# sangyun884/HR-VITON

Hardware: AMD Instinct MI355X
Metric: 1024x768 try-on images/sec (train_generator.py step: tocg+glue, G fwd/bwd, D fwd/bwd x2, VGG, Adam) (higher is better)
Workload: dtype bf16; 1 GPU; BASELINE configs[3] (SURVEY 8d config #4, headline): train_generator.py 1024x768, 4 img/GPU, --fp16 (bf16 MFMA operands, fp32 accumulate), SPADE ng...; global_batch=4, height=1024, width=768, parallelism=dp1-allreduce, persistent_grid_cus=256, dist_backend=none (single process), world_size=1, rccl_ranks=0

## Files before the change

hr-viton_amd/_lib.py:

```python
from __future__ import annotations

import ctypes as C
import os

HERE = os.path.dirname(os.path.abspath(__file__))
LIB_PATH = os.path.join(HERE, "libhrviton_hip.so")

HRV_MAX_SRC = 4
ACT_NONE, ACT_RELU, ACT_LRELU, ACT_TANH = 0, 1, 2, 3


class hrv_src_t(C.Structure):
    _fields_ = [("ptr", C.c_void_p), ("C", C.c_int32), ("cstride", C.c_int32), ("coff", C.c_int32),
                ("up_shift", C.c_int32), ("pre_act", C.c_int32), ("C_real", C.c_int32)]


class hrv_spade_epi_t(C.Structure):
    _fields_ = [("x", C.c_void_p), ("x_cstride", C.c_int32), ("x_coff", C.c_int32), ("C", C.c_int32),
                ("_pad", C.c_int32), ("mean", C.c_void_p), ("rstd", C.c_void_p), ("noise_z", C.c_void_p),
                ("noise_scale", C.c_void_p), ("g1p_out", C.c_void_p)]


class hrv_norm_bwd_t(C.Structure):
    _fields_ = [("N", C.c_int32), ("H", C.c_int32), ("W", C.c_int32), ("C", C.c_int32),
# ... 60 lines not shown
                ("act", C.c_int32), ("act_slope", C.c_float),
                ("out", C.c_void_p), ("out_cstride", C.c_int32), ("out_coff", C.c_int32),
                ("actv", C.c_void_p), ("actv_cstride", C.c_int32), ("actv_coff", C.c_int32),
                ("x_up_channels", C.c_int32), ("x2", C.c_void_p), ("x2_cstride", C.c_int32), ("x2_coff", C.c_int32),
                ("tiles", C.c_void_p), ("gb_table", C.c_void_p), ("tiles_phase", C.c_int32)]


class hrv_conv_p2_t(C.Structure):
    _fields_ = [("N", C.c_int32), ("H", C.c_int32), ("W", C.c_int32), ("Cin", C.c_int32),
                ("src", C.c_void_p), ("src_cstride", C.c_int32), ("src_coff", C.c_int32), ("Cout", C.c_int32),
                ("w_packed", C.c_void_p), ("bias", C.c_void_p),
                ("act", C.c_int32), ("act_slope", C.c_float),
                ("mask", C.c_void_p), ("mask_cstride", C.c_int32), ("mask_coff", C.c_int32), ("mask_slope", C.c_float), ("out_f32", C.c_int32),
                ("out", C.c_void_p), ("out_cstride", C.c_int32), ("out_coff", C.c_int32),
                ("res_f32", C.c_int32), ("residual", C.c_void_p), ("res_cstride", C.c_int32), ("res_coff", C.c_int32),
                ("res_after_mask", C.c_int32)]


class hrv_conv_s2_t(C.Structure):
    _fields_ = [("mode", C.c_int32),
                ("N", C.c_int32), ("Hs", C.c_int32), ("Ws", C.c_int32), ("K", C.c_int32),
                ("src", C.c_void_p), ("src_cstride", C.c_int32), ("src_coff", C.c_int32),
                ("Ho", C.c_int32), ("Wo", C.c_int32), ("cols", C.c_int32), ("Cph", C.c_int32),
                ("w_packed", C.c_void_p), ("bias", C.c_void_p),
                ("act", C.c_int32), ("act_slope", C.c_float),
                ("out", C.c_void_p), ("out_cstride", C.c_int32), ("out_coff", C.c_int32), ("out_f32", C.c_int32),
                ("residual", C.c_void_p), ("res_cstride", C.c_int32), ("res_coff", C.c_int32), ("res_f32", C.c_int32),
                ("mask", C.c_void_p), ("mask_cstride", C.c_int32), ("mask_coff", C.c_int32), ("mask_slope", C.c_float)]


class hrv_s2_pack_job_t(C.Structure):
# ... 217 lines not shown
    "hrv_grid_sample_nchw_bwd_f32": (C.c_int, [_vp, _i32, _i32, _i32, _i32, _vp, _i32, _i32, _vp, _vp, _vp, _vp]),
    "hrv_softmax_nchw_f32": (C.c_int, [_vp, _i32, _i32, _i64, _vp, _vp]),
    "hrv_softmax_nchw_bwd_f32": (C.c_int, [_vp, _vp, _i32, _i32, _i64, _vp, _vp]),
    "hrv_cross_entropy_nchw_f32": (C.c_int, [_vp, _vp, _i32, _i32, _i64, _f, _vp, _vp, _vp, _vp]),
    "hrv_tapsum_bwd_nhwc_f32": (C.c_int, [_vp, _i32, _i32, _i32, _i32, _i32, _i32, _i32, _i32, _vp, _i32, _vp]),
    "hrv_tap_expand_nhwc": (C.c_int, [_vp, _i32, _i32, _i32, _i32, _i32, _i32, _i32, _i32, _i32, _i32, _vp, _vp]),
    "hrv_mul_f32": (C.c_int, [_vp, _vp, _i64, _vp, _vp]),
    "hrv_spade_gb_packed_bytes": (_i64, [_i32, _i32, _i32, _i32]),
    "hrv_spade_gb_supported": (C.c_int, [_i32, _i32, _i32, _i32, _i32, _i32, _i32]),
    "hrv_spade_gb_pack_dev": (C.c_int, [_i32, _vp, _vp, _i32, _i32, _i32, _vp, _vp]),
    "hrv_spade_gb_bf16": (C.c_int, [C.POINTER(hrv_spade_gb_t), _vp]),
    "hrv_conv_p2_packed_bytes": (C.c_int64, [_i32, _i32]),
    "hrv_conv_p2_supported": (C.c_int, [_i32, _i32, _i32, _i32, _i32]),
    "hrv_conv_p2_pack_dev": (C.c_int, [_i32, _vp, _vp, _i32, _i32, _vp, _f, _vp, _vp]),
    "hrv_conv_p2_bf16": (C.c_int, [C.POINTER(hrv_conv_p2_t), _vp]),
    "hrv_conv_s2_packed_bytes": (C.c_int64, [_i32, _i32, _i32]),
    "hrv_conv_s2_supported": (C.c_int, [_i32, _i32, _i32, _i32, _i32, _i32, _i32]),
    "hrv_conv_s2_pack_dev": (C.c_int, [_i32, _vp, _i32, _i32, _i32, _vp, _f, _vp, _vp]),
    "hrv_conv_s2_pack_multi_dev": (C.c_int, [_i32, C.POINTER(hrv_s2_pack_job_t), _vp]),
    "hrv_conv_s2_bf16": (C.c_int, [C.POINTER(hrv_conv_s2_t), _vp]),
    "hrv_space_to_depth2_cells_bf16": (C.c_int, [_vp, _i32, _i32, _i32, _i32, _i32, _i32, _i32, _i32, _i32, _vp, _vp]),
    "hrv_instnorm_apply_nhwc_bf16out": (C.c_int, [_vp, _i32, _i32, _i32, _i32, _i32, _i32, _vp, _vp, _i32, _f, _vp, _i32, _i32, _vp]),
    "hrv_scale_bf16": (C.c_int, [_vp, _i64, _f, _vp, _vp]),
    "hrv_split3_nhwc_bf16": (C.c_int, [_vp, _i64, _i32, _i32, _i32, _vp, _vp]),
    "hrv_pad_width_nhwc_bf16": (C.c_int, [_vp, _i64, _i32, _i32, _i32, _vp, _vp]),
    "hrv_spade_fused_packed_bytes": (C.c_int64, [_i32]),
    "hrv_spade_fused_supported": (C.c_int, [_i32, _i32, _i32, _i32, _i32, _i32]),
    "hrv_spade_fused_pack_dev": (C.c_int, [_vp, _vp, _i32, _vp, _vp, _i32, _vp, _vp]),
    "hrv_spade_fused_bf16": (C.c_int, [C.POINTER(hrv_spade_fused_t), _vp]),
    "hrv_spade_tiles_plan_bytes": (C.c_int64, [_i32, _i32, _i32]),
# ... 62 lines not shown
```

hr-viton_amd/csrc/conv_p2.hip:

```cpp
#include <string.h>

#include <type_traits>
#include <utility>

#include "patch_pass.h"

namespace hrv {

constexpr int P2_PW = 20;
constexpr int P2_PBUF = 23 * 1024;
constexpr int p2_sb(int ntp) { return ntp * 2048; }
constexpr int p2_patch_off(int ntp) { return 3 * p2_sb(ntp); }
constexpr int p2_cb_off(int ntp) { return p2_patch_off(ntp) + 2 * P2_PBUF; }
constexpr int p2_lds(int ntp) { return p2_cb_off(ntp) + 512; }
constexpr int p2_blocks_per_cu(int ntp) { return ntp == 1 ? 3 : 2; }
static_assert(2 * ((p2_lds(4) + 1279) / 1280) * 1280 <= 160 * 1024, "two blocks per CU");
static_assert(3 * ((p2_lds(1) + 1279) / 1280) * 1280 <= 160 * 1024, "three blocks per CU for single-tile passes");

struct P2Params {
  const void* src; int src_cs, src_co, Cin; unsigned src_bytes;
  int N, H, W;
  const void* wp; unsigned w_bytes;
  int npass;
  int ntp[PATCH_MAXP];
// ... 99 lines not shown
  const rsrc_t a_rsrc = make_rsrc(reinterpret_cast<const char*>(p.src) + (size_t)T.n * p.src_bytes, p.src_bytes);
  const rsrc_t w_rsrc = make_rsrc(p.wp, p.w_bytes);
#pragma unroll
  for (int k = 0; k < 6; ++k) p2_patch_piece<NTP>(p, smem, a_rsrc, T, 0, 0, k * 4 + wave, lane);
#pragma unroll
  for (int q = 0; q < 2; ++q)
#pragma unroll
    for (int k = 0; k < NBW; ++k) {
      int idx = wave + 4 * k;
      idx = idx < NPW ? idx : (NPW >= 4 ? idx - 4 : idx % NPW);
      dma16(w_rsrc, reinterpret_cast<float*>(smem + q * p2_sb(NTP) + idx * 1024), (unsigned)lane * 16u,
            p.woff[pass] + (unsigned)q * (unsigned)(NPW * 1024) + (unsigned)idx * 1024u);
    }
}

template <int NTP, int EPI>
__device__ __forceinline__ void p2_pass(const P2Params& p, unsigned char* const smem, const int pass, const PatchTile T, const int bid,
                                        const bool load_consts, const bool wait_all, const bool first, const bool last, const int nxt_pass,
                                        const PatchTile NT_) {
  const int tid = threadIdx.x, lane = tid & 63;
  const int wave = __builtin_amdgcn_readfirstlane(tid >> 6);
  const int l31 = lane & 31, lh = lane >> 5;
  constexpr int NPW = NTP * 2;
  constexpr int NBW = (NPW + 3) / 4;
  constexpr int NST = 4 * NTP;
  unsigned char* const ring = smem;
  float* const cbuf = reinterpret_cast<float*>(smem + p2_cb_off(NTP));
  const rsrc_t w_rsrc = make_rsrc(p.wp, p.w_bytes);
  const rsrc_t a_rsrc = make_rsrc(reinterpret_cast<const char*>(p.src) + (size_t)T.n * p.src_bytes, p.src_bytes);
  const unsigned wbase = p.woff[pass];
  const int tile0 = p.tile0[pass];
// ... 269 lines not shown
  }
  if (p.tlog && tid == 0 && last) {
    p.tlog[(size_t)bid * 8 + 7] = tl_pack;
    p.tlog[(size_t)bid * 8 + 6] = wall_clock64();
  }
}

template <int NTP, int EPI>
__global__ __launch_bounds__(256, p2_blocks_per_cu(NTP)) void conv_p2_kernel(const P2Params p, const int pass0, const int pass1) {
  __shared__ __attribute__((aligned(1024))) unsigned char smem[p2_lds(NTP)];
  const int lane = threadIdx.x & 63, wave = __builtin_amdgcn_readfirstlane((int)threadIdx.x >> 6);
#define P2_TILE(BID) patch_tile(BID, p.W, p.H, p.m_tiles)
#define P2_HEAD(PASS, T) p2_head<NTP>(p, PASS, smem, T, wave, lane)
#define P2_PASS(...) p2_pass<NTP, EPI>(p, smem, __VA_ARGS__)
  PATCH_PASS_UNITS(p, pass0, pass1, P2_TILE, P2_HEAD, P2_PASS, p.tlog)
#undef P2_TILE
#undef P2_HEAD
#undef P2_PASS
}

}

using namespace hrv;

extern "C" int64_t hrv_conv_p2_packed_bytes(int32_t Cin, int32_t Cout) {
  PatchPlan pl;
  if (!p2_plan(Cin, Cout, pl)) return -1;
  return pl.bytes;
}

// ... 42 lines not shown
  memset(&p, 0, sizeof(p));
  p.src = d->src; p.src_cs = d->src_cstride; p.src_co = d->src_coff; p.Cin = d->Cin; p.src_bytes = (unsigned)sbytes;
  p.N = d->N; p.H = d->H; p.W = d->W;
  p.wp = d->w_packed; p.w_bytes = (unsigned)pl.bytes;
  patch_plan_copy(p, pl);
  p.nchunk = (d->Cin + 31) / 32;
  p.m_tiles = (int)patch_tiles(d->N, d->H, d->W);
  p.Cout = d->Cout;
  p.bias = d->bias; p.act = d->act; p.slope = d->act_slope;
  p.res = d->residual; p.res_cs = d->res_cstride; p.res_co = d->res_coff; p.res_f32 = d->res_f32; p.res_after = d->res_after_mask;
  p.mask = d->mask; p.mask_cs = d->mask_cstride; p.mask_co = d->mask_coff; p.mask_slope = d->mask_slope;
  p.out = d->out; p.out_cs = d->out_cstride; p.out_co = d->out_coff; p.out_f32 = d->out_f32;
  p.tlog = diag_tlog(p.m_tiles);
  p.pp = patch_pp(p.m_tiles) ? 1 : 0;
  if (p.pp) p.tlog = nullptr;
  patch_pass_groups(pl, p.m_tiles, p.pp != 0, p2_blocks_per_cu, [&](const int a, const int b, const int grid) {
    const dim3 g3(grid), b3(256);
    const hipStream_t st = (hipStream_t)stream;
    const int epi = p.res ? 2 : (p.mask ? 1 : 0);
#define P2_LAUNCH(NTP_)                                                                                                 \
  {                                                                                                                     \
    if (epi == 0) hipLaunchKernelGGL((conv_p2_kernel<NTP_, 0>), g3, b3, 0, st, p, a, b);                                \
    else if (epi == 1) hipLaunchKernelGGL((conv_p2_kernel<NTP_, 1>), g3, b3, 0, st, p, a, b);                           \
    else hipLaunchKernelGGL((conv_p2_kernel<NTP_, 2>), g3, b3, 0, st, p, a, b);                                         \
  }
    if (pl.ntp[a] == 4) P2_LAUNCH(4)
    else if (pl.ntp[a] == 3) P2_LAUNCH(3)
    else if (pl.ntp[a] == 2) P2_LAUNCH(2)
    else P2_LAUNCH(1)
#undef P2_LAUNCH
// ... 4 lines not shown
```

hr-viton_amd/gen_train.py:

```python
from __future__ import annotations

import os
from typing import Dict, List, Optional, Sequence, Tuple

import torch
import torch.nn as nn

from . import _lib, ops
from . import train_ops as T
from .ops import ACT_LRELU, ACT_NONE, ACT_RELU, ACT_TANH, Act, _ceil4

Grads = Dict[nn.Parameter, torch.Tensor]


def attach_grad_sync(sync):
    for p in sync.params:
        p._hrv_grad_sync = sync


def detach_grad_sync(params):
    for p in params:
        if hasattr(p, "_hrv_grad_sync"):
            del p._hrv_grad_sync

# ... 200 lines not shown

    def forward(self, x: Act, actv: Optional[Act], z: Optional[torch.Tensor], save: bool = True, fused=None, stats=None):
        n = self.norm
        dev = x.t.device
        if fused is not None:
            sg, shift = fused
            zz = z
            if stats is not None:
                ns, (mean, rstd) = stats
            else:
                ns = self.vecs()[1] if zz is not None else None
                mean, rstd = ops.instnorm_stats(x, zz, ns if zz is not None else None)
            out = ops.alloc(x.N, x.H, x.W, self.C, dev, bf16=True)
            g1p = torch.empty((x.N, x.H, x.W, self.Cp), dtype=torch.bfloat16, device=dev) if save else None
            pk = T.spade_fused_pack(self.shared.wparam.data, self.shared.bparam.data, n.conv_gamma.weight.data, n.conv_beta.weight.data)
            T.spade_fused_forward(sg, shift, x, mean, rstd, zz, n.noise_scale.data, pk, n.conv_gamma.bias.data, n.conv_beta.bias.data,
                                  self.act, 0.2, out, g1p, actv if save else None, self.name + ".conv_shared+gamma|beta",
                                  tiles=T.spade_tile_plan_for(sg, shift, x.N, x.H, x.W))
            ctx = dict(x=x, z=zz, ns=ns, mean=mean, rstd=rstd, actv=actv, g1p=Act(g1p, self.C) if save else None, out=out)
            return out, ctx
        bc, ns = self.vecs()
        zz = z
        if stats is not None:
            mean, rstd = stats[1]
        else:
            mean, rstd = ops.instnorm_stats(x, zz, ns if zz is not None else None)
        mb = T.MMA_BF16[0]
        cfg = ops.engine_tile("mb", 0, self.G * 64, mb and actv.bf16, 3, 3, 1, 1, 1, 0, self.hid, x.N, x.H, x.W, wide=True,
                              base=None if mb else self.cfg)
        out_bf16 = mb and actv.bf16 and self.C % 8 == 0
        if (mb and actv.bf16 and out_bf16 and x.cstride % 4 == 0 and
                T.spade_gb_ok(0, self.C, self.Cp, self.hid, x.N, x.H, x.W)):
            out = ops.alloc(x.N, x.H, x.W, self.C, dev, bf16=True)
            g1p = torch.empty((x.N, x.H, x.W, self.Cp), dtype=torch.bfloat16, device=dev) if save else None
# ... 85 lines not shown
        with T.wgrad_side(dgb.N * dgb.H * dgb.W, dgb, actv):
            dwcat, db = _pair_slot(n.conv_gamma.weight, n.conv_beta.weight), _pair_slot(n.conv_gamma.bias, n.conv_beta.bias)
            if Cp != C_ or dwcat is None or db is None:
                dwcat = torch.empty((2 * Cp, self.hid, 3, 3), device=dev)
                db = torch.empty(2 * Cp, device=dev)
            T.conv_wgrad(dgb, actv, 0, 0, self.hid, 3, 3, 1, 1, dwcat, name=self.name + ".gb.wgrad", dbias=db)
            direct = flat_grad_slot(n.conv_gamma.weight) is not None
            keep = (lambda t: t) if direct else (lambda t: t.clone())
            _acc(grads, n.conv_gamma.weight, keep(dwcat[:C_]))
            _acc(grads, n.conv_beta.weight, keep(dwcat[Cp:Cp + C_]))
            _acc(grads, n.conv_gamma.bias, keep(db[:C_]))
            _acc(grads, n.conv_beta.bias, keep(db[Cp:Cp + C_]))
        if (Cp == C_ and T.MMA_BF16[0] and dgb.bf16 and actv.bf16 and dact.cstride % 8 == 0 and (2 * C_) % 32 == 0 and
                T.conv_p2_ok(2 * C_, self.hid, actv.N, actv.H, actv.W)):
            pk = T.conv_p2_pack(2, n.conv_gamma.weight.data, n.conv_beta.weight.data, 2 * C_, self.hid)
            T.conv_p2(dgb, pk, self.hid, dact, mask=actv, mask_slope=0.0, name=self.name + ".gb.dgrad",
                      flops=2.0 * actv.N * actv.H * actv.W * 2 * C_ * self.hid * 9, tag=" [spade_gb]")
        elif (Cp == C_ and T.MMA_BF16[0] and dgb.bf16 and actv.bf16 and
                T.spade_gb_ok(1, C_, Cp, self.hid, actv.N, actv.H, actv.W)):
            T.spade_gb_dgrad(dgb, T.spade_gb_pack(1, n.conv_gamma.weight.data, n.conv_beta.weight.data), C_, actv, 0.0, dact,
                             self.name + ".gb.dgrad")
        else:
            T.conv_dgrad(dgb, wcat, actv.H, actv.W, 1, 1, act_mask=actv, slope=0.0, out=dact, name=self.name + ".gb.dgrad",
                         batch=getattr(self.shared, "pack_batch", None) if Cp == C_ else None)


class BlockT:
    def __init__(self, blk: nn.Module, name: str):
        self.blk, self.name = blk, name
        self.learned = blk.learned_shortcut
        self.n0 = SpadeT(blk.norm_0, ACT_LRELU, name + ".norm_0")
        self.n1 = SpadeT(blk.norm_1, ACT_LRELU, name + ".norm_1")
# ... 38 lines not shown
        mb = T.MMA_BF16[0] and (seg.W >> seg_shift) % 4 == 0
        sg = seg
        if mb and seg.coff == 0 and seg.cstride == 8:
            sg = getattr(seg, "_as_bf16", None)
            if sg is None:
                sg = seg._as_bf16 = Act(seg.t.to(torch.bfloat16), seg.C)
        mb = mb and sg.bf16
        segx = ops.tap_expand(sg, seg_shift, 3)
        cp = sg.Cp
        wt_all, b_all = T.shared_taps_prep([n_.shared.wparam.data for n_ in norms], [n_.shared.bparam.data for n_ in norms], cp)
        hid = norms[0].hid
        actv_all = T.conv_forward_dev(wt_all, [(segx, 0)], 1, 0, shift=b_all, act=ACT_RELU,
                                      out_bf16=mb, name=self.name + ".conv_shared[x%d as 1x1 over taps]" % len(norms))
        return segx, [actv_all.slice(hid * i, hid) for i in range(len(norms))]

    def shared_backward(self, segx: Act, dact_all: Act, grads: Grads):
        norms = self.norms()
        hid, cp = norms[0].hid, segx.C // 9
        with T.wgrad_side(dact_all.N * dact_all.H * dact_all.W, dact_all, segx):
            dw = torch.empty((hid * len(norms), segx.C, 1, 1), device=dact_all.t.device)
            db = torch.empty(hid * len(norms), device=dact_all.t.device)
            T.conv_wgrad(dact_all, segx, 0, 0, segx.C, 1, 1, 1, 0, dw, name=self.name + ".conv_shared.wgrad", dbias=db)
            gws = [grad_buffer(n_.shared.wparam) for n_ in norms]
            gbs = [grad_buffer(n_.shared.bparam) for n_ in norms]
            T.shared_taps_grad(dw, db, gws, gbs, cp)
            for n_, gw, gb in zip(norms, gws, gbs):
                _acc(grads, n_.shared.wparam, gw)
                _acc(grads, n_.shared.bparam, gb)

    def forward(self, x: Act, seg: Act, seg_shift: int, zs, out: Optional[Act], out_up: int, out_act: int,
                save: bool = True):
        zi = iter(zs)
        ctx = {"x": x}
        sgf = self.fused_label_map(x, seg, seg_shift)
        fused = None
        if sgf is not None:
            fused = (sgf, seg_shift)
            norms = self.norms()
            hid = norms[0].hid
# ... 23 lines not shown
        h0, ctx["n0"] = self.n0.forward(x, next(ai), z_0, save, fused, st_0)
        dx = self.c0.forward([(h0, 0)])
        h1, ctx["n1"] = self.n1.forward(dx, next(ai), next(zi), save, fused)
        o = self.c1.forward([(h1, 0)], residual=x_s, act=out_act, out=out, out_up=out_up,
                            out_bf16=out is None and h1.bf16 and self.c1.conv.out_channels % 8 == 0)
        ctx.update(h0=h0, h1=h1)
        return o, ctx

    def backward(self, ctx, d_out: Act, grads: Grads) -> Act:
        x = ctx["x"]
        norms = self.norms()
        hid = norms[0].hid
        dact_all = ops.alloc(x.N, x.H, x.W, hid * len(norms), x.t.device,
                             bf16=bool(T.MMA_BF16[0] and ctx["segx"].bf16 and x.W % 4 == 0))
        k0 = 1 if self.learned else 0
        dh16 = bool(T.MMA_BF16[0] and os.environ.get("HRV_DH_BF16", "1") != "0")
        def down(conv, d_y, h, norm, nctx):
            slot = norm.dout_slot(nctx, dh16 and h.bf16)
            if slot is None:
                return conv.backward(d_y, [(h, 0)], grads, dx_bf16=dh16 and h.bf16), None
            dgb, dbeta, mask = slot
            conv.backward(d_y, [(h, 0)], grads, act_mask=mask, slope=0.2, dx_out=dbeta)
            return dbeta, dgb
        d_h1, dgb1 = down(self.c1, d_out, ctx["h1"], self.n1, ctx["n1"])
        d_dx = self.n1.backward(ctx["n1"], d_h1, grads, None, False, dact_all.slice(hid * (k0 + 1), hid), dx_bf16=True, dgb=dgb1)
        d_h0, dgb0 = down(self.c0, d_dx, ctx["h0"], self.n0, ctx["n0"])
        mode = os.environ.get("HRV_NORM_BWD2", "")
        d_hs = None
        if self.learned and mode != "0" and ctx["n0"]["z"] is not None and ctx["ns"]["z"] is not None and not x.bf16:
            d_hs, dgbs = down(self.cs, d_out, ctx["hs"], self.ns_, ctx["ns"])
            a0, as_ = self.n0.norm_args(ctx["n0"], d_h0), self.ns_.norm_args(ctx["ns"], d_hs)
            for a, dgb in ((a0, dgb0), (as_, dgbs)):
                if dgb is not None:
                    a.update(act=ACT_NONE, out=None, dgb=dgb)
            pair = T.norm_bwd2(x, a0, as_, only_where_faster=mode != "1")
            if pair is not None:
                d_x, dgb0, dgbs = pair
                self.n0.after_norm(ctx["n0"], dgb0, a0["dnoise_scale"], grads, dact_all.slice(hid * k0, hid))
                self.ns_.after_norm(ctx["ns"], dgbs, as_["dnoise_scale"], grads, dact_all.slice(0, hid))
                self.shared_backward(ctx["segx"], dact_all, grads)
                return d_x
        d_x = self.n0.backward(ctx["n0"], d_h0, grads, None, False, dact_all.slice(hid * k0, hid), dgb=dgb0)
        if self.learned:
            if d_hs is None:
                d_hs, dgbs = down(self.cs, d_out, ctx["hs"], self.ns_, ctx["ns"])
            self.ns_.backward(ctx["ns"], d_hs, grads, d_x, True, dact_all.slice(0, hid), dgb=dgbs)
        else:
            T.add_slice(d_out, d_x, True)
        self.shared_backward(ctx["segx"], dact_all, grads)
        return d_x


def noise_elems(gen: nn.Module, N: int) -> int:
    return sum((3 if getattr(gen, name).learned_shortcut else 2) * ((N * (gen.sw << j) * (gen.sh << j) + 3) // 4 * 4)
               for j, name in enumerate(gen._blocks()))


def noise_planes(gen: nn.Module, N: int, zall: torch.Tensor):
    out, off = {}, 0
    for j, name in enumerate(gen._blocks()):
        h, w = gen.sh << j, gen.sw << j
        zn = N * w * h
        planes = []
        for _ in range(3 if getattr(gen, name).learned_shortcut else 2):
# ... 723 lines not shown
```

hr-viton_amd/train_ops.py:

```python
from __future__ import annotations

import ctypes as C
import itertools
import os
from typing import Optional, Sequence, Tuple

import torch

from . import _lib, ops
from .conv_dispatch import (COUT1, MMA_BF16, P2, THIN, conv_p2_ok, plan_dgrad, plan_forward,
                            plan_wgrad, wgrad_desc)
from .ops import ACT_LRELU, ACT_NONE, ACT_RELU, Act, _ceil4, _stream, _Timed, _workspace


_FROZEN_PACKS: dict = {}


def evict_serving_packs(tokens):
    toks = set(tokens)
    dead = [k for k in _FROZEN_PACKS
            if any(isinstance(e, tuple) and len(e) == 3 and e[0] == "serve" and e[1] in toks for e in k)]
    for k in dead:
        del _FROZEN_PACKS[k]
    return len(dead)
# ... 1591 lines not shown
    nbytes = lib.hrv_conv_p2_packed_bytes(K, cols)
    assert nbytes > 0, (K, cols)
    buf = torch.empty(nbytes // 2, dtype=torch.bfloat16, device=w.device)
    _lib.check(lib.hrv_conv_p2_pack_dev(mode, w.data_ptr(), None if w2 is None else w2.data_ptr(), K, cols,
                                        None if sigma is None else sigma.data_ptr(), wscale, buf.data_ptr(), _stream()),
               "hrv_conv_p2_pack_dev")
    if key is not None:
        if len(_FROZEN_PACKS) > 256:
            _FROZEN_PACKS.clear()
        _FROZEN_PACKS[key] = (buf, ())
    return buf


def conv_p2(src: Act, packed: torch.Tensor, cols: int, out: Act, bias: Optional[torch.Tensor] = None, act: int = ACT_NONE, slope: float = 0.2,
            mask: Optional[Act] = None, mask_slope: float = 0.0, name: str = "conv", flops: float = 0.0, tag: str = "",
            residual: Optional[Act] = None, res_after_mask: bool = False, variant: str = ""):
    lib = _lib.load()
    assert src.bf16 and out.C == cols
    d = _lib.hrv_conv_p2_t()
    d.N, d.H, d.W, d.Cin = src.N, src.H, src.W, src.C
    d.src, d.src_cstride, d.src_coff, d.Cout = src.t.data_ptr(), src.cstride, src.coff, cols
    d.w_packed = packed.data_ptr()
    if bias is not None:
        d.bias = bias.data_ptr()
    d.act, d.act_slope = act, slope
    if mask is not None:
        assert mask.bf16 and mask.C == cols
        d.mask, d.mask_cstride, d.mask_coff, d.mask_slope = mask.t.data_ptr(), mask.cstride, mask.coff, mask_slope
    d.out, d.out_cstride, d.out_coff, d.out_f32 = out.t.data_ptr(), out.cstride, out.coff, 0 if out.bf16 else 1
    if residual is not None:
        assert residual.C == cols
        d.residual, d.res_cstride, d.res_coff, d.res_f32 = residual.t.data_ptr(), residual.cstride, residual.coff, 0 if residual.bf16 else 1
        d.res_after_mask = 1 if res_after_mask else 0
    nb = (ops.act_bytes(src) + ops.act_bytes(out) + (ops.act_bytes(mask) if mask is not None else 0.0) +
          (ops.act_bytes(residual) if residual is not None else 0.0) + 2.0 * src.C * cols * 9)
    with ops._Timed("conv", name + tag, flops, nb, "conv_p2_kernel", variant):
        _lib.check(lib.hrv_conv_p2_bf16(C.byref(d), _stream()), f"hrv_conv_p2_bf16[{name}]")
    return out


S2_FWD, S2_DGRAD, S2_CELLS = 0, 1, 2


def conv_s2_ok(mode: int, K: int, cols: int, Cph: int, N: int, Ho: int, Wo: int) -> bool:
    if os.environ.get("HRV_CONV_S2", "1") == "0":
        return False
    return bool(_lib.load().hrv_conv_s2_supported(mode, K, cols, Cph, N, Ho, Wo))


def conv_s2_pack(mode: int, w: torch.Tensor, K: int, cols: int, Cph: int = 0, sigma: Optional[torch.Tensor] = None,
                 wscale: float = 1.0, split3: bool = False) -> torch.Tensor:
    lib = _lib.load()
    assert w.is_contiguous() and w.dtype == torch.float32
# ... 104 lines not shown
```

include/hrviton_hip.h:

```cpp
#ifndef HRVITON_HIP_H
#define HRVITON_HIP_H

#include <stddef.h>
#include <stdint.h>

#ifdef __cplusplus
extern "C" {
#endif

typedef void* hrv_stream_t;

enum hrv_status {
  HRV_OK = 0,
  HRV_ERR_ARG = -1,
  HRV_ERR_LAUNCH = -2,
  HRV_ERR_NODEV = -3
};

enum hrv_act { HRV_ACT_NONE = 0, HRV_ACT_RELU = 1, HRV_ACT_LRELU = 2, HRV_ACT_TANH = 3 };

const char* hrv_version(void);
const char* hrv_last_error(void);
int hrv_device_check(void);
int hrv_set_reserved_cus(int32_t k);
// ... 534 lines not shown
int64_t hrv_spade_tiles_plan_bytes(int32_t N, int32_t H, int32_t W);
int hrv_spade_tiles_bf16(const void* seg, int32_t seg_H, int32_t seg_W, int32_t seg_shift, int32_t N, int32_t H, int32_t W,
                         void* plan, hrv_stream_t stream);

typedef struct hrv_conv_p2 {
  int32_t N, H, W, Cin;
  const void* src; int32_t src_cstride, src_coff, Cout;
  const void* w_packed;
  const float* bias;
  int32_t act; float act_slope;
  const void* mask; int32_t mask_cstride, mask_coff; float mask_slope; int32_t out_f32;
  void* out; int32_t out_cstride, out_coff;
  int32_t res_f32;
  const void* residual; int32_t res_cstride, res_coff;
  int32_t res_after_mask;
} hrv_conv_p2_t;
int64_t hrv_conv_p2_packed_bytes(int32_t Cin, int32_t Cout);
int hrv_conv_p2_supported(int32_t Cin, int32_t Cout, int32_t N, int32_t H, int32_t W);
int hrv_conv_p2_pack_dev(int32_t mode, const float* w, const float* w2, int32_t Cin, int32_t Cout, const float* sigma, float wscale,
                         void* out, hrv_stream_t stream);
int hrv_conv_p2_bf16(const hrv_conv_p2_t* d, hrv_stream_t stream);

typedef struct hrv_conv_s2 {
  int32_t mode;
  int32_t N, Hs, Ws, K;
  const void* src; int32_t src_cstride, src_coff;
  int32_t Ho, Wo, cols, Cph;
  const void* w_packed;
  const float* bias;
  int32_t act; float act_slope;
  void* out; int32_t out_cstride, out_coff, out_f32;
  const void* residual; int32_t res_cstride, res_coff, res_f32;
  const void* mask; int32_t mask_cstride, mask_coff; float mask_slope;
} hrv_conv_s2_t;
#define HRV_S2_SPLIT3 4
int64_t hrv_conv_s2_packed_bytes(int32_t mode, int32_t K, int32_t cols);
// ... 80 lines not shown
```

Before: 64.75 images/s.

## Skip SPADE gamma/beta dgrad on uniform-label tiles using tile sums

SPADE backward now reuses the forward tile plan so the gamma/beta dgrad conv runs only over heavy (non-uniform segmentation) tiles. For light tiles, whose segmentation label is uniform, it zeroes dact and computes per-label windowed sums of dgb. A small apply kernel then folds those sums into the shared conv's weight and bias gradients analytically. The aim is to avoid full conv work on the many uniform tiles at high resolution, at the cost of extra kernels, a workspace buffer and more complex gradient bookkeeping.

```diff
diff --git a/hr-viton_amd/_lib.py b/hr-viton_amd/_lib.py
--- a/hr-viton_amd/_lib.py
+++ b/hr-viton_amd/_lib.py
@@ -98,7 +98,17 @@
                 ("mask", C.c_void_p), ("mask_cstride", C.c_int32), ("mask_coff", C.c_int32), ("mask_slope", C.c_float), ("out_f32", C.c_int32),
                 ("out", C.c_void_p), ("out_cstride", C.c_int32), ("out_coff", C.c_int32),
                 ("res_f32", C.c_int32), ("residual", C.c_void_p), ("res_cstride", C.c_int32), ("res_coff", C.c_int32),
-                ("res_after_mask", C.c_int32)]
+                ("res_after_mask", C.c_int32), ("tiles", C.c_void_p)]
+
+
+class hrv_spade_light_t(C.Structure):
+    _fields_ = [("N", C.c_int32), ("H", C.c_int32), ("W", C.c_int32), ("C", C.c_int32),
+                ("plan", C.c_void_p),
+                ("dgb", C.c_void_p), ("dgb_cstride", C.c_int32), ("dgb_coff", C.c_int32),
+                ("dact", C.c_void_p), ("dact_cstride", C.c_int32), ("dact_coff", C.c_int32),
+                ("hid", C.c_int32), ("_pad", C.c_int32),
+                ("workspace", C.c_void_p), ("workspace_bytes", C.c_int64),
+                ("sums", C.c_void_p)]
 
 
 class hrv_conv_s2_t(C.Structure):
@@ -346,6 +356,9 @@
     "hrv_conv_p2_supported": (C.c_int, [_i32, _i32, _i32, _i32, _i32]),
     "hrv_conv_p2_pack_dev": (C.c_int, [_i32, _vp, _vp, _i32, _i32, _vp, _f, _vp, _vp]),
     "hrv_conv_p2_bf16": (C.c_int, [C.POINTER(hrv_conv_p2_t), _vp]),
+    "hrv_spade_light_workspace_bytes": (C.c_int64, [_i32, _i32, _i32, _i32]),
+    "hrv_spade_light_sums_bf16": (C.c_int, [C.POINTER(hrv_spade_light_t), _vp]),
+    "hrv_spade_light_apply_f32": (C.c_int, [_vp, _vp, _vp, _i32, _i32, _vp, _i32, _i32, _vp, _i32, _i32, _i32, _vp, _i32, _i32, _i32, _vp, _vp]),
     "hrv_conv_s2_packed_bytes": (C.c_int64, [_i32, _i32, _i32]),
     "hrv_conv_s2_supported": (C.c_int, [_i32, _i32, _i32, _i32, _i32, _i32, _i32]),
     "hrv_conv_s2_pack_dev": (C.c_int, [_i32, _vp, _i32, _i32, _i32, _vp, _f, _vp, _vp]),
diff --git a/hr-viton_amd/csrc/conv_p2.hip b/hr-viton_amd/csrc/conv_p2.hip
--- a/hr-viton_amd/csrc/conv_p2.hip
+++ b/hr-viton_amd/csrc/conv_p2.hip
@@ -4,6 +4,7 @@
 #include <utility>
 
 #include "patch_pass.h"
+#include "spade_tiles.h"
 
 namespace hrv {
 
@@ -137,7 +138,7 @@
     }
 }
 
-template <int NTP, int EPI>
+template <int NTP, int EPI, bool LIST = false>
 __device__ __forceinline__ void p2_pass(const P2Params& p, unsigned char* const smem, const int pass, const PatchTile T, const int bid,
                                         const bool load_consts, const bool wait_all, const bool first, const bool last, const int nxt_pass,
                                         const PatchTile NT_) {
@@ -437,6 +438,22 @@
 #define P2_HEAD(PASS, T) p2_head<NTP>(p, PASS, smem, T, wave, lane)
 #define P2_PASS(...) p2_pass<NTP, EPI>(p, smem, __VA_ARGS__)
   PATCH_PASS_UNITS(p, pass0, pass1, P2_TILE, P2_HEAD, P2_PASS, p.tlog)
+#undef P2_TILE
+#undef P2_HEAD
+#undef P2_PASS
+}
+
+typedef const __attribute__((address_space(4))) int* p2_cint_p;
+template <int NTP, int EPI>
+__global__ __launch_bounds__(256, p2_blocks_per_cu(NTP)) void conv_p2_list_kernel(const P2Params p, const int pass0, const int pass1,
+                                                                                 const int* const tplan) {
+  __shared__ __attribute__((aligned(1024))) unsigned char smem[p2_lds(NTP)];
+  const int lane = threadIdx.x & 63, wave = __builtin_amdgcn_readfirstlane((int)threadIdx.x >> 6);
+  struct { int pp, m_tiles; } sch = {p.pp, ((p2_cint_p)tplan)[ST_NHEAVY]};
+#define P2_TILE(BID) patch_tile_at(((p2_cint_p)tplan)[ST_HDR + xcd_remap(BID, sch.m_tiles)] & ST_TILE_MASK, p.W, p.H)
+#define P2_HEAD(PASS, T) p2_head<NTP>(p, PASS, smem, T, wave, lane)
+#define P2_PASS(...) p2_pass<NTP, EPI, true>(p, smem, __VA_ARGS__)
+  PATCH_PASS_UNITS(sch, pass0, pass1, P2_TILE, P2_HEAD, P2_PASS, p.tlog)
 #undef P2_TILE
 #undef P2_HEAD
 #undef P2_PASS
@@ -509,6 +526,14 @@
   p.tlog = diag_tlog(p.m_tiles);
   p.pp = patch_pp(p.m_tiles) ? 1 : 0;
   if (p.pp) p.tlog = nullptr;
+  if (d->tiles) {
+    HRV_REQUIRE(pl.npass == 1 && pl.ntp[0] == 4 && p.mask && !p.res && p.m_tiles < ST_MAX_TILES && ((uintptr_t)d->tiles & 3) == 0,
+                "conv_p2: a tile plan goes with 128 columns, a mask and no residual");
+    const int cap = p2_blocks_per_cu(4) * persistent_cus();
+    hipLaunchKernelGGL((conv_p2_list_kernel<4, 1>), dim3(p.m_tiles < cap ? p.m_tiles : cap), dim3(256), 0, (hipStream_t)stream, p, 0, 1,
+                       (const int*)d->tiles);
+    return check_launch("conv_p2_list_kernel");
+  }
   patch_pass_groups(pl, p.m_tiles, p.pp != 0, p2_blocks_per_cu, [&](const int a, const int b, const int grid) {
     const dim3 g3(grid), b3(256);
     const hipStream_t st = (hipStream_t)stream;
diff --git a/hr-viton_amd/csrc/spade_light.hip b/hr-viton_amd/csrc/spade_light.hip
--- /dev/null
+++ b/hr-viton_amd/csrc/spade_light.hip
@@ -0,0 +1,209 @@
+#include "patch_pass.h"
+#include "spade_tiles.h"
+
+namespace hrv {
+
+struct SlParams {
+  const unsigned short* dgb; int dgb_cs, dgb_co, C2;
+  unsigned short* dact; int dact_cs, dact_co, hid;
+  int N, H, W, m_tiles;
+  const int* plan;
+  float* ws;
+  float* sums;
+};
+
+constexpr int SL_CH = 112;
+
+__global__ __launch_bounds__(256, 4) void spade_light_sums_kernel(const SlParams p) {
+  __shared__ float colsum[3][18][SL_CH];
+  const int nl = p.plan[ST_NLIGHT];
+  const int* const light = p.plan + ST_HDR + p.m_tiles;
+  const int tid = threadIdx.x;
+  const int HG = p.hid >> 3;
+  for (int u = blockIdx.x; u < nl; u += gridDim.x) {
+    const PatchTile T = patch_tile_at(light[u] & ST_TILE_MASK, p.W, p.H);
+    for (int idx = tid; idx < 256 * HG; idx += 256) {
+      const int pix = idx / HG, g = idx - pix * HG;
+      const size_t pidx = ((size_t)T.n * p.H + T.y0 + (pix >> 4)) * p.W + T.x0 + (pix & 15);
+      *reinterpret_cast<uint4*>(p.dact + pidx * p.dact_cs + p.dact_co + 8 * g) = make_uint4(0u, 0u, 0u, 0u);
+    }
+    const unsigned short* const patch = p.dgb + (((size_t)T.n * p.H + T.y0 - 1) * p.W + T.x0 - 1) * p.dgb_cs + p.dgb_co;
+#pragma unroll 1
+    for (int c0 = 0; c0 < p.C2; c0 += SL_CH) {
+      const int nch = p.C2 - c0 < SL_CH ? p.C2 - c0 : SL_CH, ng = nch >> 3;
+      __syncthreads();
+#pragma unroll 1
+      for (int item = tid; item < 18 * ng; item += 256) {
+        const int x = item / ng, g = item - x * ng;
+        const unsigned src = (unsigned)((x * p.dgb_cs + c0 + 8 * g) * 2);
+        float r[3][8];
+#pragma unroll
+        for (int i = 0; i < 3; ++i)
+#pragma unroll
+          for (int e = 0; e < 8; ++e) r[i][e] = 0.f;
+        const unsigned rstride = (unsigned)(p.W * p.dgb_cs * 2);
+#pragma unroll
+        for (int yb = 0; yb < 18; yb += 6) {
+          uint4 v[6];
+#pragma unroll
+          for (int i = 0; i < 6; ++i) v[i] = *reinterpret_cast<const uint4*>(reinterpret_cast<const char*>(patch) + (src + (unsigned)(yb + i) * rstride));
+#pragma unroll
+          for (int i = 0; i < 6; ++i) {
+            const int y = yb + i;
+            const unsigned w[4] = {v[i].x, v[i].y, v[i].z, v[i].w};
+#pragma unroll
+            for (int e = 0; e < 8; ++e) {
+              const float f = __builtin_bit_cast(float, (e & 1) ? (w[e >> 1] & 0xFFFF0000u) : (w[e >> 1] << 16));
+              if (y <= 15) r[0][e] += f;
+              if (y >= 1 && y <= 16) r[1][e] += f;
+              if (y >= 2) r[2][e] += f;
+            }
+          }
+          asm volatile("" ::: "memory");
+        }
+#pragma unroll
+        for (int i = 0; i < 3; ++i)
+#pragma unroll
+          for (int e = 0; e < 8; ++e) colsum[i][x][8 * g + e] = r[i][e];
+      }
+      __syncthreads();
+#pragma unroll 1
+      for (int item = tid; item < 9 * nch; item += 256) {
+        const int wd = item / nch, c = item - wd * nch;
+        const int ry = wd / 3, rx = wd - 3 * ry;
+        float s = 0.f;
+#pragma unroll
+        for (int x = 0; x < 16; ++x) s += colsum[ry][rx + x][c];
+        p.ws[((size_t)u * 9 + (2 - ry) * 3 + (2 - rx)) * p.C2 + c0 + c] = s;
+      }
+    }
+  }
+}
+
+__global__ __launch_bounds__(256) void spade_light_reduce_kernel(const SlParams p) {
+  __shared__ float red[16][8][16];
+  const int nl = p.plan[ST_NLIGHT];
+  const int* const light = p.plan + ST_HDR + p.m_tiles;
+  const int il = threadIdx.x & 15, sl = threadIdx.x >> 4;
+  const int items = 9 * p.C2;
+  const int item = blockIdx.x * 16 + il;
+  const int u0 = (int)(((long long)nl * sl) / 16), u1 = (int)(((long long)nl * (sl + 1)) / 16);
+  float acc[8];
+#pragma unroll
+  for (int k = 0; k < 8; ++k) acc[k] = 0.f;
+  if (item < items)
+    for (int u = u0; u < u1; ++u) {
+      const int k = light[u] >> 24;
+      const float v = p.ws[(size_t)u * items + item];
+#pragma unroll
+      for (int e = 0; e < 8; ++e) acc[e] += e == k ? v : 0.f;
+    }
+#pragma unroll
+  for (int k = 0; k < 8; ++k) red[sl][k][il] = acc[k];
+  __syncthreads();
+  if (threadIdx.x < 128) {
+    const int k = threadIdx.x >> 4, i = blockIdx.x * 16 + il;
+    float s = 0.f;
+#pragma unroll
+    for (int q = 0; q < 16; ++q) s += red[q][k][il];
+    if (i < items) p.sums[(size_t)k * items + i] = s;
+  }
+}
+
+struct SlApplyParams {
+  const float* sums;
+  const float* wg;
+  const float* wb;
+  int C, hid;
+  const unsigned short* actv; int actv_cs, actv_co;
+  int H, W;
+  const int* plan;
+  float* dw; int K, cp, row0;
+  float* db;
+};
+
+#pragma clang fp contract(off)
+__global__ __launch_bounds__(256) void spade_light_apply_kernel(const SlApplyParams p) {
+  __shared__ float red[32][8];
+  const int cl = threadIdx.x & 7, part = threadIdx.x >> 3;
+  const int c = blockIdx.x * 8 + cl;
+  const int C2 = 2 * p.C;
+  float dbacc = 0.f;
+  for (int k = 0; k < 8; ++k) {
+    const int rep = p.plan[ST_REP + k];
+    if (rep < 0) continue;
+    float s = 0.f;
+    if (c < p.hid)
+      for (int o = part; o < C2; o += 32) {
+        const float* const w = (o < p.C ? p.wg + (size_t)o * p.hid * 9 : p.wb + (size_t)(o - p.C) * p.hid * 9) + (size_t)c * 9;
+#pragma unroll
+        for (int t = 0; t < 9; ++t) s += static_cast<float>(static_cast<__bf16>(w[t])) * p.sums[((size_t)k * 9 + t) * C2 + o];
+      }
+    __syncthreads();
+    red[part][cl] = s;
+    __syncthreads();
+    if (part == 0 && c < p.hid) {
+      float D = 0.f;
+#pragma unroll
+      for (int q = 0; q < 32; ++q) D += red[q][cl];
+      const PatchTile R = patch_tile_at(rep, p.W, p.H);
+      const short a = (short)p.actv[(((size_t)R.n * p.H + R.y0) * p.W + R.x0) * p.actv_cs + p.actv_co + c];
+      if (a > 0) {
+        float* const row = p.dw + (size_t)(p.row0 + c) * p.K + k;
+#pragma unroll
+        for (int t = 0; t < 9; ++t) row[t * p.cp] += D;
+        dbacc += D;
+      }
+    }
+  }
+  if (part == 0 && c < p.hid) p.db[p.row0 + c] += dbacc;
+}
+
+}
+
+using namespace hrv;
+
+extern "C" int64_t hrv_spade_light_workspace_bytes(int32_t N, int32_t H, int32_t W, int32_t C) {
+  if (N <= 0 || H <= 0 || W <= 0 || C <= 0 || patch_tiles(N, H, W) >= ST_MAX_TILES) return -1;
+  return patch_tiles(N, H, W) * 9 * 2 * (int64_t)C * 4;
+}
+
+extern "C" int hrv_spade_light_sums_bf16(const hrv_spade_light_t* d, hrv_stream_t stream) {
+  HRV_REQUIRE(d != nullptr && d->plan && d->dgb && d->dact && d->workspace && d->sums, "spade_light_sums: null pointer");
+  HRV_REQUIRE(d->N > 0 && d->H > 0 && d->W > 0 && patch_tiles(d->N, d->H, d->W) < ST_MAX_TILES, "spade_light_sums: bad extent");
+  HRV_REQUIRE(d->C > 0 && d->C % 4 == 0 && d->hid > 0 && d->hid % 8 == 0, "spade_light_sums: 2 C and hid must be multiples of 8 (C %d, hid %d)", d->C,
+              d->hid);
+  HRV_REQUIRE(d->dgb_cstride % 8 == 0 && d->dgb_coff % 8 == 0 && d->dgb_coff >= 0 && d->dgb_coff + 2 * d->C <= d->dgb_cstride,
+              "spade_light_sums: dgb slice");
+  HRV_REQUIRE(d->dact_cstride % 8 == 0 && d->dact_coff % 8 == 0 && d->dact_coff >= 0 && d->dact_coff + d->hid <= d->dact_cstride,
+              "spade_light_sums: dact slice");
+  HRV_REQUIRE((((uintptr_t)d->dgb | (uintptr_t)d->dact | (uintptr_t)d->workspace | (uintptr_t)d->sums) & 15) == 0 && ((uintptr_t)d->plan & 3) == 0,
+              "spade_light_sums: alignment");
+  HRV_REQUIRE(19 * (int64_t)d->W * d->dgb_cstride * 2 < (int64_t)0xFFFFFFF0, "spade_light_sums: 18 rows of dgb exceed the 32-bit offsets of a patch");
+  HRV_REQUIRE(d->workspace_bytes >= hrv_spade_light_workspace_bytes(d->N, d->H, d->W, d->C), "spade_light_sums: workspace too small");
+  SlParams p;
+  p.dgb = (const unsigned short*)d->dgb; p.dgb_cs = d->dgb_cstride; p.dgb_co = d->dgb_coff; p.C2 = 2 * d->C;
+  p.dact = (unsigned short*)d->dact; p.dact_cs = d->dact_cstride; p.dact_co = d->dact_coff; p.hid = d->hid;
+  p.N = d->N; p.H = d->H; p.W = d->W; p.m_tiles = (int)patch_tiles(d->N, d->H, d->W);
+  p.plan = (const int*)d->plan; p.ws = d->workspace; p.sums = d->sums;
+  const int cap = 4 * persistent_cus();
+  hipLaunchKernelGGL(spade_light_sums_kernel, dim3(p.m_tiles < cap ? p.m_tiles : cap), dim3(256), 0, (hipStream_t)stream, p);
+  hipLaunchKernelGGL(spade_light_reduce_kernel, dim3((9 * p.C2 + 15) / 16), dim3(256), 0, (hipStream_t)stream, p);
+  return check_launch("spade_light_sums");
+}
+
+extern "C" int hrv_spade_light_apply_f32(const float* sums, const float* w_gamma, const float* w_beta, int32_t C, int32_t hid, const void* actv,
+                                         int32_t actv_cstride, int32_t actv_coff, const void* plan, int32_t N, int32_t H, int32_t W, float* dw,
+                                         int32_t rows, int32_t row0, int32_t cp, float* db, hrv_stream_t stream) {
+  HRV_REQUIRE(sums && w_gamma && w_beta && actv && plan && dw && db, "spade_light_apply: null pointer");
+  HRV_REQUIRE(N > 0 && H > 0 && W > 0 && patch_tiles(N, H, W) < ST_MAX_TILES && C > 0 && hid > 0, "spade_light_apply: bad extent");
+  HRV_REQUIRE(cp >= 8 && row0 >= 0 && row0 + hid <= rows, "spade_light_apply: rows %d .. %d of %d, %d label channels per tap", row0, row0 + hid, rows, cp);
+  HRV_REQUIRE(actv_coff >= 0 && actv_coff + hid <= actv_cstride, "spade_light_apply: actv slice");
+  SlApplyParams p;
+  p.sums = sums; p.wg = w_gamma; p.wb = w_beta; p.C = C; p.hid = hid;
+  p.actv = (const unsigned short*)actv; p.actv_cs = actv_cstride; p.actv_co = actv_coff;
+  p.H = H; p.W = W; p.plan = (const int*)plan;
+  p.dw = dw; p.K = 9 * cp; p.cp = cp; p.row0 = row0; p.db = db;
+  hipLaunchKernelGGL(spade_light_apply_kernel, dim3((hid + 7) / 8), dim3(256), 0, (hipStream_t)stream, p);
+  return check_launch("spade_light_apply_kernel");
+}
diff --git a/hr-viton_amd/gen_train.py b/hr-viton_amd/gen_train.py
--- a/hr-viton_amd/gen_train.py
+++ b/hr-viton_amd/gen_train.py
@@ -238,10 +238,12 @@
             out = ops.alloc(x.N, x.H, x.W, self.C, dev, bf16=True)
             g1p = torch.empty((x.N, x.H, x.W, self.Cp), dtype=torch.bfloat16, device=dev) if save else None
             pk = T.spade_fused_pack(self.shared.wparam.data, self.shared.bparam.data, n.conv_gamma.weight.data, n.conv_beta.weight.data)
+            tiles = T.spade_tile_plan_for(sg, shift, x.N, x.H, x.W)
             T.spade_fused_forward(sg, shift, x, mean, rstd, zz, n.noise_scale.data, pk, n.conv_gamma.bias.data, n.conv_beta.bias.data,
                                   self.act, 0.2, out, g1p, actv if save else None, self.name + ".conv_shared+gamma|beta",
-                                  tiles=T.spade_tile_plan_for(sg, shift, x.N, x.H, x.W))
-            ctx = dict(x=x, z=zz, ns=ns, mean=mean, rstd=rstd, actv=actv, g1p=Act(g1p, self.C) if save else None, out=out)
+                                  tiles=tiles)
+            ctx = dict(x=x, z=zz, ns=ns, mean=mean, rstd=rstd, actv=actv, g1p=Act(g1p, self.C) if save else None, out=out,
+                       tiles=tiles if save else None)
             return out, ctx
         bc, ns = self.vecs()
         zz = z
@@ -357,8 +359,12 @@
         if (Cp == C_ and T.MMA_BF16[0] and dgb.bf16 and actv.bf16 and dact.cstride % 8 == 0 and (2 * C_) % 32 == 0 and
                 T.conv_p2_ok(2 * C_, self.hid, actv.N, actv.H, actv.W)):
             pk = T.conv_p2_pack(2, n.conv_gamma.weight.data, n.conv_beta.weight.data, 2 * C_, self.hid)
+            tiles = T.spade_bwd_tile_plan(ctx.get("tiles")) if dact.bf16 and dgb.C == 2 * C_ and self.hid % 8 == 0 else None
+            ctx["light_sums"] = None
+            if tiles is not None:
+                ctx["light_sums"] = (T.spade_light_sums(dgb, tiles, dact, self.name + ".gb.dgrad"), tiles)
             T.conv_p2(dgb, pk, self.hid, dact, mask=actv, mask_slope=0.0, name=self.name + ".gb.dgrad",
-                      flops=2.0 * actv.N * actv.H * actv.W * 2 * C_ * self.hid * 9, tag=" [spade_gb]")
+                      flops=2.0 * actv.N * actv.H * actv.W * 2 * C_ * self.hid * 9, tag=" [spade_gb]", tiles=tiles)
         elif (Cp == C_ and T.MMA_BF16[0] and dgb.bf16 and actv.bf16 and
                 T.spade_gb_ok(1, C_, Cp, self.hid, actv.N, actv.H, actv.W)):
             T.spade_gb_dgrad(dgb, T.spade_gb_pack(1, n.conv_gamma.weight.data, n.conv_beta.weight.data), C_, actv, 0.0, dact,
@@ -427,7 +433,7 @@
                                       out_bf16=mb, name=self.name + ".conv_shared[x%d as 1x1 over taps]" % len(norms))
         return segx, [actv_all.slice(hid * i, hid) for i in range(len(norms))]
 
-    def shared_backward(self, segx: Act, dact_all: Act, grads: Grads):
+    def shared_backward(self, segx: Act, dact_all: Act, grads: Grads, nctxs=()):
         norms = self.norms()
         hid, cp = norms[0].hid, segx.C // 9
         with T.wgrad_side(dact_all.N * dact_all.H * dact_all.W, dact_all, segx):
@@ -436,6 +442,11 @@
             T.conv_wgrad(dact_all, segx, 0, 0, segx.C, 1, 1, 1, 0, dw, name=self.name + ".conv_shared.wgrad", dbias=db)
             gws = [grad_buffer(n_.shared.wparam) for n_ in norms]
             gbs = [grad_buffer(n_.shared.bparam) for n_ in norms]
+            for j, (n_, nctx) in enumerate(zip(norms, nctxs)):
+                light = nctx.get("light_sums")
+                if light is not None:
+                    T.spade_light_apply(light[0], n_.norm.conv_gamma.weight.data, n_.norm.conv_beta.weight.data, nctx["actv"], light[1],
+                                        dw, db, hid * j, cp, n_.name + ".conv_shared.wgrad")
             T.shared_taps_grad(dw, db, gws, gbs, cp)
             for n_, gw, gb in zip(norms, gws, gbs):
                 _acc(grads, n_.shared.wparam, gw)
@@ -489,6 +500,7 @@
         dact_all = ops.alloc(x.N, x.H, x.W, hid * len(norms), x.t.device,
                              bf16=bool(T.MMA_BF16[0] and ctx["segx"].bf16 and x.W % 4 == 0))
         k0 = 1 if self.learned else 0
+        nctxs = ([ctx["ns"]] if self.learned else []) + [ctx["n0"], ctx["n1"]]
         dh16 = bool(T.MMA_BF16[0] and os.environ.get("HRV_DH_BF16", "1") != "0")
         def down(conv, d_y, h, norm, nctx):
             slot = norm.dout_slot(nctx, dh16 and h.bf16)
@@ -513,7 +525,7 @@
                 d_x, dgb0, dgbs = pair
                 self.n0.after_norm(ctx["n0"], dgb0, a0["dnoise_scale"], grads, dact_all.slice(hid * k0, hid))
                 self.ns_.after_norm(ctx["ns"], dgbs, as_["dnoise_scale"], grads, dact_all.slice(0, hid))
-                self.shared_backward(ctx["segx"], dact_all, grads)
+                self.shared_backward(ctx["segx"], dact_all, grads, nctxs)
                 return d_x
         d_x = self.n0.backward(ctx["n0"], d_h0, grads, None, False, dact_all.slice(hid * k0, hid), dgb=dgb0)
         if self.learned:
@@ -522,7 +534,7 @@
             self.ns_.backward(ctx["ns"], d_hs, grads, d_x, True, dact_all.slice(0, hid), dgb=dgbs)
         else:
             T.add_slice(d_out, d_x, True)
-        self.shared_backward(ctx["segx"], dact_all, grads)
+        self.shared_backward(ctx["segx"], dact_all, grads, nctxs)
         return d_x
 
 
diff --git a/hr-viton_amd/train_ops.py b/hr-viton_amd/train_ops.py
--- a/hr-viton_amd/train_ops.py
+++ b/hr-viton_amd/train_ops.py
@@ -1629,7 +1629,7 @@
 
 def conv_p2(src: Act, packed: torch.Tensor, cols: int, out: Act, bias: Optional[torch.Tensor] = None, act: int = ACT_NONE, slope: float = 0.2,
             mask: Optional[Act] = None, mask_slope: float = 0.0, name: str = "conv", flops: float = 0.0, tag: str = "",
-            residual: Optional[Act] = None, res_after_mask: bool = False, variant: str = ""):
+            residual: Optional[Act] = None, res_after_mask: bool = False, variant: str = "", tiles: Optional[SpadeTilePlan] = None):
     lib = _lib.load()
     assert src.bf16 and out.C == cols
     d = _lib.hrv_conv_p2_t()
@@ -1649,9 +1649,60 @@
         d.res_after_mask = 1 if res_after_mask else 0
     nb = (ops.act_bytes(src) + ops.act_bytes(out) + (ops.act_bytes(mask) if mask is not None else 0.0) +
           (ops.act_bytes(residual) if residual is not None else 0.0) + 2.0 * src.C * cols * 9)
+    if tiles is not None:
+        assert (tiles.N, tiles.H, tiles.W) == (src.N, src.H, src.W), "tile plan of another level"
+        d.tiles = tiles.ws.data_ptr()
+        if ops._Prof.enabled:
+            fh = tiles.counts()[0] / float(tiles.tiles)
+            wbytes = 2.0 * src.C * cols * 9
+            flops, nb = flops * fh, (nb - wbytes) * fh + wbytes
     with ops._Timed("conv", name + tag, flops, nb, "conv_p2_kernel", variant):
         _lib.check(lib.hrv_conv_p2_bf16(C.byref(d), _stream()), f"hrv_conv_p2_bf16[{name}]")
     return out
+
+
+def spade_bwd_tile_plan(tiles: Optional[SpadeTilePlan]) -> Optional[SpadeTilePlan]:
+    if tiles is None or os.environ.get("HRV_SPADE_UNIFORM_BWD", "1") == "0":
+        return None
+    try:
+        min_tiles = max(1, int(os.environ.get("HRV_SPADE_UNIFORM_BWD_MIN_TILES", "4096")))
+    except ValueError:
+        min_tiles = 4096
+    return tiles if tiles.tiles >= min_tiles else None
+
+
+def spade_light_sums(dgb: Act, tiles: SpadeTilePlan, dact: Act, name: str = "spade") -> torch.Tensor:
+    lib = _lib.load()
+    assert dgb.bf16 and dact.bf16 and dgb.C % 8 == 0 and (tiles.N, tiles.H, tiles.W) == (dgb.N, dgb.H, dgb.W)
+    C_ = dgb.C // 2
+    d = _lib.hrv_spade_light_t()
+    d.N, d.H, d.W, d.C = dgb.N, dgb.H, dgb.W, C_
+    d.plan = tiles.ws.data_ptr()
+    d.dgb, d.dgb_cstride, d.dgb_coff = dgb.t.data_ptr(), dgb.cstride, dgb.coff
+    d.dact, d.dact_cstride, d.dact_coff, d.hid = dact.t.data_ptr(), dact.cstride, dact.coff, dact.C
+    nbytes = lib.hrv_spade_light_workspace_bytes(dgb.N, dgb.H, dgb.W, C_)
+    assert nbytes > 0, (dgb.N, dgb.H, dgb.W, C_)
+    ws = torch.empty(nbytes // 4, dtype=torch.float32, device=dgb.t.device)
+    sums = torch.empty(8 * 9 * 2 * C_, dtype=torch.float32, device=dgb.t.device)
+    d.workspace, d.workspace_bytes, d.sums = ws.data_ptr(), nbytes, sums.data_ptr()
+    nb = 0.0
+    if ops._Prof.enabled:
+        nb = tiles.counts()[1] * (324.0 * dgb.C * 2 + 256.0 * dact.C * 2)
+    with ops._Timed("conv", name + " [uniform tiles]", 0.0, nb, "spade_light_sums_kernel"):
+        _lib.check(lib.hrv_spade_light_sums_bf16(C.byref(d), _stream()), "hrv_spade_light_sums_bf16")
+    return sums
+
+
+def spade_light_apply(sums: torch.Tensor, w_gamma: torch.Tensor, w_beta: torch.Tensor, actv: Act, tiles: SpadeTilePlan, dw: torch.Tensor,
+                      db: torch.Tensor, row0: int, cp: int, name: str = "spade"):
+    lib = _lib.load()
+    C_, hid = w_gamma.shape[0], w_gamma.shape[1]
+    assert w_gamma.is_contiguous() and w_beta.is_contiguous() and tuple(w_beta.shape) == tuple(w_gamma.shape) == (C_, hid, 3, 3)
+    assert actv.bf16 and actv.C == hid and dw.is_contiguous() and db.is_contiguous() and dw.shape[1] == 9 * cp and sums.numel() == 144 * C_
+    with ops._Timed("conv", name + " [uniform tiles]", 0.0, 4.0 * (2 * C_ * hid * 9 + 144 * C_), "spade_light_apply_kernel"):
+        _lib.check(lib.hrv_spade_light_apply_f32(sums.data_ptr(), w_gamma.data_ptr(), w_beta.data_ptr(), C_, hid, actv.t.data_ptr(), actv.cstride,
+                                                 actv.coff, tiles.ws.data_ptr(), actv.N, actv.H, actv.W, dw.data_ptr(), dw.shape[0], row0, cp,
+                                                 db.data_ptr(), _stream()), "hrv_spade_light_apply_f32")
 
 
 S2_FWD, S2_DGRAD, S2_CELLS = 0, 1, 2
diff --git a/include/hrviton_hip.h b/include/hrviton_hip.h
--- a/include/hrviton_hip.h
+++ b/include/hrviton_hip.h
@@ -572,12 +572,28 @@
   int32_t res_f32;
   const void* residual; int32_t res_cstride, res_coff;
   int32_t res_after_mask;
+  const void* tiles;
 } hrv_conv_p2_t;
 int64_t hrv_conv_p2_packed_bytes(int32_t Cin, int32_t Cout);
 int hrv_conv_p2_supported(int32_t Cin, int32_t Cout, int32_t N, int32_t H, int32_t W);
 int hrv_conv_p2_pack_dev(int32_t mode, const float* w, const float* w2, int32_t Cin, int32_t Cout, const float* sigma, float wscale,
                          void* out, hrv_stream_t stream);
 int hrv_conv_p2_bf16(const hrv_conv_p2_t* d, hrv_stream_t stream);
+
+typedef struct hrv_spade_light {
+  int32_t N, H, W, C;
+  const void* plan;
+  const void* dgb; int32_t dgb_cstride, dgb_coff;
+  void* dact; int32_t dact_cstride, dact_coff;
+  int32_t hid, _pad;
+  float* workspace; int64_t workspace_bytes;
+  float* sums;
+} hrv_spade_light_t;
+int64_t hrv_spade_light_workspace_bytes(int32_t N, int32_t H, int32_t W, int32_t C);
+int hrv_spade_light_sums_bf16(const hrv_spade_light_t* d, hrv_stream_t stream);
+int hrv_spade_light_apply_f32(const float* sums, const float* w_gamma, const float* w_beta, int32_t C, int32_t hid, const void* actv,
+                              int32_t actv_cstride, int32_t actv_coff, const void* plan, int32_t N, int32_t H, int32_t W, float* dw,
+                              int32_t rows, int32_t row0, int32_t cp, float* db, hrv_stream_t stream);
 
 typedef struct hrv_conv_s2 {
   int32_t mode;
```

Result: no change. 65.23 images/s, median of 6 (+0.7%).
